# ChenFengYe/motion-latent-diffusion

Hardware: NVIDIA H100
Metric: motions/sec @ 50-step DDIM text-to-motion, batch 256 (higher is better)
Workload: dtype f16x2-split (fp32-equivalent, fp32 accumulate)

## Files before the change

mld_b200/csrc/gemm_tc.cu:

```cuda
#include "gemm_tc.h"

#include <algorithm>

#include "tc_common.cuh"

namespace {
using namespace tc;

constexpr int BM = 128, BK = 64;
constexpr int NUM_THREADS = 384;
constexpr int MMA_THREADS = 256;
constexpr int CONSUMER_WARPS = 8;
constexpr int MAX_N = 1024;
constexpr int MAX_N_WIDE = 4096;

struct TcParams {
  int M, N, kblocks, kb1;
  int m_tiles, n_tiles;
  float inv_scale;
  const float* bias;
  const float* addtab;
  int act;
  __half* out_hi; __half* out_lo; int ld_out, out_col0;
  float* out_f32; int ldc;
// ... 348 lines not shown
};

__global__ void __launch_bounds__(MMA_THREADS, 1)
k_ffn_tc(const __grid_constant__ CUtensorMap tmXh, const __grid_constant__ CUtensorMap tmXl,
         const __grid_constant__ CUtensorMap tmW1h, const __grid_constant__ CUtensorMap tmW1l,
         const __grid_constant__ CUtensorMap tmW2h, const __grid_constant__ CUtensorMap tmW2l,
         const __grid_constant__ CUtensorMap tmAh, const __grid_constant__ CUtensorMap tmAl,
         const __grid_constant__ CUtensorMap tmWoh, const __grid_constant__ CUtensorMap tmWol,
         const __grid_constant__ CUtensorMap tmYh, const __grid_constant__ CUtensorMap tmYl, const FfnParams p) {
  using Cfg = FfnCfg;
  constexpr int STAGES = Cfg::STAGES;
  extern __shared__ uint8_t smem_raw[];
  uint8_t* smem = smem_raw + smem_pad1024(smem_raw);
  uint8_t* ring = smem + Cfg::X_BYTES;
  uint64_t* bar_full = reinterpret_cast<uint64_t*>(ring + STAGES * Cfg::STAGE_BYTES);
  uint64_t* bar_empty = bar_full + STAGES;
  uint64_t* bar_xfull = bar_empty + STAGES;
  uint64_t* bar_xempty = bar_xfull + 4;

  const int warp = __shfl_sync(0xffffffffu, (int)(threadIdx.x >> 5), 0), lane = threadIdx.x & 31;
  int tl_n = 0;
  tl_event(p.tl, tl_n, 40);
  const int ncta = (int)gridDim.x, cid = (int)blockIdx.x;
  const int NC = p.n_chunks;
  struct Item { int mt, c0, c1, mode, piece0; };
  auto rev = [&](int t) { return p.reverse ? p.m_tiles - 1 - t : t; };
  const int nlocal = p.full + (cid < p.left * p.parts ? 1 : 0);
  auto item = [&](int j) -> Item {
    if (j < p.full) return Item{rev(cid + j * ncta), 0, NC, 0, 0};
    const int t = cid / p.parts, part = cid - t * p.parts;
    const int c0 = (part * NC + p.parts - 1) / p.parts, c1 = ((part + 1) * NC + p.parts - 1) / p.parts;
    const int slot0 = t * (p.parts - 1);
    return Item{rev(p.full * ncta + t), c0, c1, p.parts == 1 ? 0 : (part == p.parts - 1 ? 2 : 1),
                p.parts == 1 ? 0 : slot0 + (part == p.parts - 1 ? 0 : part)};
  };
  const int PRE = p.prefix ? 8 : 0;
  const int per_tile = PRE + 4 * NC;
  int total = p.full * per_tile;
  if (nlocal > p.full) {
    const Item it = item(p.full);
    total += PRE + 4 * (it.c1 - it.c0);
  }
  const int XG = p.prefix ? 2 : 1;
  const int xtotal = nlocal * 4 * XG;

  if (threadIdx.x == 0) {
    for (int s = 0; s < STAGES; ++s) {
      mbar_init(smem_u32(&bar_full[s]), 1);
      mbar_init(smem_u32(&bar_empty[s]), CONSUMER_WARPS);
    }
    for (int kb = 0; kb < 4; ++kb) {
      mbar_init(smem_u32(&bar_xfull[kb]), 1);
      mbar_init(smem_u32(&bar_xempty[kb]), CONSUMER_WARPS);
    }
    asm volatile("fence.mbarrier_init.release.cluster;" ::: "memory");
    tma_prefetch_desc(&tmXh); tma_prefetch_desc(&tmXl); tma_prefetch_desc(&tmW1h);
    tma_prefetch_desc(&tmW1l); tma_prefetch_desc(&tmW2h); tma_prefetch_desc(&tmW2l);
    tma_prefetch_desc(&tmYh); tma_prefetch_desc(&tmYl);
    if (p.prefix) { tma_prefetch_desc(&tmAh); tma_prefetch_desc(&tmAl); tma_prefetch_desc(&tmWoh); tma_prefetch_desc(&tmWol); }
  }
  pdl_trigger();
  __syncthreads();
  pdl_wait();
  tl_event(p.tl, tl_n, 41);

  int q_next = 0, x_next = 0;
  auto load_slot = [&](int q) {
    const int j = min(q / per_tile, p.full);
    const Item it = item(j);
    const int r = q - j * per_tile;
    if (elect_one()) {
      const uint32_t full = smem_u32(&bar_full[q % STAGES]);
      const uint32_t dst = smem_u32(ring + (q % STAGES) * Cfg::STAGE_BYTES);
      mbar_expect_tx(full, Cfg::STAGE_BYTES);
      if (r < PRE) {
        tma_load_2d(dst, (r & 1) ? &tmWol : &tmWoh, full, (r >> 1) * BK, 0);
      } else {
        const int c = it.c0 + ((r - PRE) >> 2), k = (r - PRE) & 3;
        if (k < 2) {
          for (int kk = 0; kk < 2; ++kk) {
            tma_load_2d(dst + kk * 8192, &tmW1h, full, (2 * k + kk) * BK, c * Cfg::CHUNK);
            tma_load_2d(dst + 16384 + kk * 8192, &tmW1l, full, (2 * k + kk) * BK, c * Cfg::CHUNK);
          }
        } else {
          tma_load_2d(dst, k == 3 ? &tmW2l : &tmW2h, full, c * Cfg::CHUNK, 0);
        }
      }
    }
    __syncwarp();
  };
  auto load_x = [&](int v) {
    if (elect_one()) {
      const int j = v / (4 * XG), kb = v & 3;
      const bool att = p.prefix && (v >> 2) == j * XG;
      const int m0 = item(j).mt * BM;
      const uint32_t full = smem_u32(&bar_xfull[kb]);
      mbar_expect_tx(full, 2 * BM * 128);
      tma_load_2d(smem_u32(smem + kb * 16384), att ? &tmAh : &tmXh, full, kb * BK, m0);
      tma_load_2d(smem_u32(smem + 65536 + kb * 16384), att ? &tmAl : &tmXl, full, kb * BK, m0);
      if (att && kb == 0)
        for (int k2 = 0; k2 < 4; ++k2) { tma_prefetch_2d(&tmXh, k2 * BK, m0); tma_prefetch_2d(&tmXl, k2 * BK, m0); }
      if (v % (4 * XG) == 0 && j + 1 < nlocal) {
        const int m1 = item(j + 1).mt * BM;
        for (int k2 = 0; k2 < 4; ++k2) {
          tma_prefetch_2d(&tmXh, k2 * BK, m1); tma_prefetch_2d(&tmXl, k2 * BK, m1);
          if (p.prefix) { tma_prefetch_2d(&tmAh, k2 * BK, m1); tma_prefetch_2d(&tmAl, k2 * BK, m1); }
        }
      }
    }
    __syncwarp();
  };
  auto produce = [&](int need, int need_x) {
    ring_produce(x_next, xtotal, need_x, bar_xempty, 4, load_x);
    ring_produce(q_next, total, need, bar_empty, STAGES, load_slot);
  };

  const int cw = warp >> 2;
  const int cp = 2 * (lane & 3);
  const int rl = cw * 64 + (warp & 3) * 16 + (lane >> 2);
  const uint32_t sX = smem_u32(smem) + cw * (64 * 128);
  float acc2[128];
  float acc1[32];
  uint32_t hh[4][4], hl[4][4];
  int rc = 0;
  auto slot_full = [&](int r) { mbar_wait(smem_u32(&bar_full[r % STAGES]), ((uint32_t)(r / STAGES)) & 1u); };
  auto slot_free = [&](int r) { if (lane == 0) mbar_arrive(smem_u32(&bar_empty[r % STAGES])); };
  auto x_full = [&](int kb, uint32_t par) { mbar_wait(smem_u32(&bar_xfull[kb]), par); };
  auto x_free = [&](int kb) { if (lane == 0) mbar_arrive(smem_u32(&bar_xempty[kb])); };
  for (int j = 0; j < nlocal; ++j) {
    const Item it = item(j);
    const int m0 = it.mt * BM;
    const uint32_t xpar = (uint32_t)(j * XG) & 1u;
    if (warp == 0) produce(-1, 4 * j * XG + 3);
    if (p.prefix) {
#pragma unroll
      for (int kb = 0; kb < 4; ++kb) {
        if (warp == 0) produce(rc + 1, -1);
        x_full(kb, xpar);
        slot_full(rc); slot_full(rc + 1);
        const uint32_t wh = smem_u32(ring + (rc % STAGES) * Cfg::STAGE_BYTES);
        const uint32_t wl = smem_u32(ring + ((rc + 1) % STAGES) * Cfg::STAGE_BYTES);
        wg_fence();
        kblock_ss<256>(acc2, sX + kb * 16384, sX + 65536 + kb * 16384, wh, wl, kb == 0);
        wg_commit();
        wg_wait<0>();
        slot_free(rc); slot_free(rc + 1); x_free(kb);
        rc += 2;
        if (warp == 0) produce(-1, -1);
        tl_event(p.tl, tl_n, 60, kb);
      }
      acc_fence(acc2);
      if (warp == 0) produce(-1, 4 * j * XG + 7);
#pragma unroll
      for (int kb = 0; kb < 4; ++kb) x_full(kb, xpar ^ 1u);
      ln_tile(acc2, p.inv_s0, p.b0, p.gamma1, p.beta1, smem, rl, lane, cp);
      fence_async_smem();
      named_bar_sync(2 + cw, 128);
      tl_event(p.tl, tl_n, 61, j);
    } else {
#pragma unroll
      for (int kb = 0; kb < 4; ++kb) x_full(kb, xpar);
    }
    tl_event(p.tl, tl_n, 2, j);
    int pend = -1;
    for (int c = it.c0; c < it.c1; ++c) {
#pragma unroll
      for (int half = 0; half < 2; ++half) {
        if (warp == 0) produce(rc + half, -1);
        slot_full(rc + half);
        tl_event(p.tl, tl_n, 10 + half, c);
        const uint32_t w = smem_u32(ring + ((rc + half) % STAGES) * Cfg::STAGE_BYTES);
        wg_fence();
#pragma unroll
        for (int k = 0; k < 2; ++k) {
          const uint32_t xh = sX + (2 * half + k) * 16384;
          kblock_ss<64>(acc1, xh, xh + 65536, w + k * 8192, w + 16384 + k * 8192, half == 0 && k == 0);
        }
        wg_commit();
      }
      wg_wait<0>();
      acc_fence(acc1);
      tl_event(p.tl, tl_n, 13, c);
      if (pend >= 0) slot_free(pend);
      slot_free(rc); slot_free(rc + 1);
      rc += 2;
      if (c == it.c1 - 1 && it.mode == 1)
        for (int kb = 0; kb < 4; ++kb) x_free(kb);
      if (warp == 0) produce(-1, -1);
#pragma unroll
      for (int ks = 0; ks < 4; ++ks) {
#pragma unroll
        for (int g = 0; g < 2; ++g) {
          const int jj = 2 * ks + g, n = c * Cfg::CHUNK + 8 * jj + cp;
          const float2 b = p.b1 ? __ldg(reinterpret_cast<const float2*>(p.b1 + n)) : make_float2(0.0f, 0.0f);
          split2(gelu_fast(fmaf(acc1[4 * jj], p.inv_s1, b.x)), gelu_fast(fmaf(acc1[4 * jj + 1], p.inv_s1, b.y)),
                 hh[ks][2 * g], hl[ks][2 * g]);
          split2(gelu_fast(fmaf(acc1[4 * jj + 2], p.inv_s1, b.x)), gelu_fast(fmaf(acc1[4 * jj + 3], p.inv_s1, b.y)),
                 hh[ks][2 * g + 1], hl[ks][2 * g + 1]);
        }
      }
      tl_event(p.tl, tl_n, 14, c);
      if (warp == 0) produce(rc, -1);
      slot_full(rc);
      tl_event(p.tl, tl_n, 12, c);
      wg_fence();
      {
        const uint64_t wd = make_desc(smem_u32(ring + (rc % STAGES) * Cfg::STAGE_BYTES));
#pragma unroll
        for (int ks = 0; ks < 4; ++ks) {
          wgmma_rs_n256(acc2, hl[ks], wd + 2 * ks, (c == it.c0 && ks == 0) ? 0u : 1u);
          wgmma_rs_n256(acc2, hh[ks], wd + 2 * ks, 1u);
        }
      }
      wg_commit();
      if (warp == 0) produce(rc + 1, -1);
      slot_full(rc + 1);
      {
        const uint64_t wd = make_desc(smem_u32(ring + ((rc + 1) % STAGES) * Cfg::STAGE_BYTES));
#pragma unroll
        for (int ks = 0; ks < 4; ++ks) wgmma_rs_n256(acc2, hh[ks], wd + 2 * ks, 1u);
      }
      wg_commit();
      wg_wait<1>();
      slot_free(rc);
      pend = rc + 1;
      rc += 2;
      if (warp == 0) produce(-1, -1);
    }
    wg_wait<0>();
    acc_fence(acc2);
    if (pend >= 0) slot_free(pend);
    if (warp == 0) produce(-1, -1);
    tl_event(p.tl, tl_n, 4, j);
    if (it.mode == 1) {
      float* const dst = p.scratch + (size_t)it.piece0 * (BM * 256);
#pragma unroll
      for (int jj = 0; jj < 32; ++jj) {
        *reinterpret_cast<float2*>(dst + rl * 256 + 8 * jj + cp) = make_float2(acc2[4 * jj], acc2[4 * jj + 1]);
        *reinterpret_cast<float2*>(dst + (rl + 8) * 256 + 8 * jj + cp) = make_float2(acc2[4 * jj + 2], acc2[4 * jj + 3]);
      }
      __threadfence();
      named_bar_sync(1, MMA_THREADS);
      if (threadIdx.x == 0) asm volatile("st.release.gpu.global.u32 [%0], %1;" ::"l"(p.flags + it.piece0), "r"(1) : "memory");
      continue;
    }
    const int nparts = it.mode == 2 ? p.parts - 1 : 0;
    if (nparts > 0) {
      if (lane == 0) {
        for (int pp = 0; pp < nparts; ++pp) {
          const int* f = p.flags + it.piece0 + pp;
          uint32_t v = 0;
          long long t_end = clock64() + 4000000000ll;
          do {
            asm volatile("ld.acquire.gpu.global.u32 %0, [%1];" : "=r"(v) : "l"(f) : "memory");
            if (v == 0 && clock64() > t_end) __trap();
          } while (v == 0);
        }
      }
      __syncwarp();
      for (int pp = 0; pp < nparts; ++pp) {
        const float* src = p.scratch + (size_t)(it.piece0 + pp) * (BM * 256);
#pragma unroll
        for (int jj = 0; jj < 32; ++jj) {
          const float2 a = __ldcg(reinterpret_cast<const float2*>(src + rl * 256 + 8 * jj + cp));
          const float2 b = __ldcg(reinterpret_cast<const float2*>(src + (rl + 8) * 256 + 8 * jj + cp));
          acc2[4 * jj] += a.x; acc2[4 * jj + 1] += a.y; acc2[4 * jj + 2] += b.x; acc2[4 * jj + 3] += b.y;
        }
      }
      named_bar_sync(1, MMA_THREADS);
      if (threadIdx.x == 0)
        for (int pp = 0; pp < nparts; ++pp) p.flags[it.piece0 + pp] = 0;
    }
    ln_tile(acc2, p.inv_s2, p.b2, p.gamma, p.beta, smem, rl, lane, cp);
    fence_async_smem();
    named_bar_sync(2 + cw, 128);
    tl_event(p.tl, tl_n, 62, j);
    if ((warp & 3) == 0) {
      if (elect_one()) {
        if (m0 + cw * 64 < p.M) {
#pragma unroll
          for (int kb = 0; kb < 4; ++kb) {
            const uint32_t src = smem_u32(smem + kb * 16384 + cw * 8192);
            tma_store_2d(&tmYh, src, kb * BK, m0 + cw * 64);
            tma_store_2d(&tmYl, src + 65536, kb * BK, m0 + cw * 64);
          }
          bulk_commit();
          bulk_wait_read<0>();
        }
#pragma unroll
        for (int kb = 0; kb < 4; ++kb) mbar_arrive_cnt(smem_u32(&bar_xempty[kb]), 4);
      }
      __syncwarp();
      tl_event(p.tl, tl_n, 63, j);
    }
  }
  tl_event(p.tl, tl_n, 42);
}

struct ProjParams {
  int M, n_chunks, items;
  float inv_scale;
  const float* bias;
  __half* out_hi; __half* out_lo; int ld_out, out_col0;
  long long* tl;
};
struct ProjCfg {
  static constexpr int CHUNK = 128;
  static constexpr int A_BYTES = 2 * 4 * BM * 128;
  static constexpr int STAGE_BYTES = 2 * CHUNK * 128, STAGES = 3;
  static constexpr int SMEM_BYTES = A_BYTES + STAGES * STAGE_BYTES + 256 + 1024;
  static_assert(SMEM_BYTES <= 232448, "shared memory budget");
};

template <int ACT>
__global__ void __launch_bounds__(MMA_THREADS, 1)
k_proj_tc(const __grid_constant__ CUtensorMap tmAh, const __grid_constant__ CUtensorMap tmAl,
          const __grid_constant__ CUtensorMap tmWh, const __grid_constant__ CUtensorMap tmWl, const ProjParams p) {
  using Cfg = ProjCfg;
  constexpr int STAGES = Cfg::STAGES;
  extern __shared__ uint8_t smem_raw[];
  uint8_t* smem = smem_raw + smem_pad1024(smem_raw);
  uint8_t* ring = smem + Cfg::A_BYTES;
  uint64_t* bar_full = reinterpret_cast<uint64_t*>(ring + STAGES * Cfg::STAGE_BYTES);
  uint64_t* bar_empty = bar_full + STAGES;
  uint64_t* bar_afull = bar_empty + STAGES;
  uint64_t* bar_aempty = bar_afull + 4;

  const int warp = __shfl_sync(0xffffffffu, (int)(threadIdx.x >> 5), 0), lane = threadIdx.x & 31;
  int tl_n = 0;
  tl_event(p.tl, tl_n, 40);
  const int NC = p.n_chunks;
  const int t0 = (int)((long long)blockIdx.x * p.items / gridDim.x);
  const int n = (int)((long long)(blockIdx.x + 1) * p.items / gridDim.x) - t0;
  const int mt0 = t0 / NC, ntiles = (t0 + n - 1) / NC - mt0 + 1;
  auto tile_of = [&](int i) { return (t0 + i) / NC - mt0; };
  auto first_of_tile = [&](int i) { return i == 0 || (t0 + i) % NC == 0; };
  auto last_of_tile = [&](int i) { return i == n - 1 || (t0 + i + 1) % NC == 0; };

  if (threadIdx.x == 0) {
    for (int s = 0; s < STAGES; ++s) {
      mbar_init(smem_u32(&bar_full[s]), 1);
      mbar_init(smem_u32(&bar_empty[s]), CONSUMER_WARPS);
    }
    for (int k = 0; k < 4; ++k) {
      mbar_init(smem_u32(&bar_afull[k]), 1);
      mbar_init(smem_u32(&bar_aempty[k]), CONSUMER_WARPS);
    }
    asm volatile("fence.mbarrier_init.release.cluster;" ::: "memory");
    tma_prefetch_desc(&tmAh); tma_prefetch_desc(&tmAl); tma_prefetch_desc(&tmWh); tma_prefetch_desc(&tmWl);
  }
  pdl_trigger();
  __syncthreads();
  pdl_wait();
  tl_event(p.tl, tl_n, 41);

  int q_next = 0, a_next = 0;
  auto load_w = [&](int q) {
    if (elect_one()) {
      const int c = (t0 + (q >> 2)) % NC, k = q & 3;
      const uint32_t full = smem_u32(&bar_full[q % STAGES]);
      const uint32_t dst = smem_u32(ring + (q % STAGES) * Cfg::STAGE_BYTES);
      mbar_expect_tx(full, Cfg::STAGE_BYTES);
      tma_load_2d(dst, &tmWh, full, k * BK, c * Cfg::CHUNK);
      tma_load_2d(dst + Cfg::STAGE_BYTES / 2, &tmWl, full, k * BK, c * Cfg::CHUNK);
    }
    __syncwarp();
  };
  auto load_a = [&](int a) {
    if (elect_one()) {
      const int j = a >> 2, k = a & 3, m0 = (mt0 + j) * BM;
      const uint32_t full = smem_u32(&bar_afull[k]);
      mbar_expect_tx(full, 2 * BM * 128);
      tma_load_2d(smem_u32(smem + k * 16384), &tmAh, full, k * BK, m0);
      tma_load_2d(smem_u32(smem + 65536 + k * 16384), &tmAl, full, k * BK, m0);
      if (k == 0 && j + 1 < ntiles)
        for (int k2 = 0; k2 < 4; ++k2) { tma_prefetch_2d(&tmAh, k2 * BK, m0 + BM); tma_prefetch_2d(&tmAl, k2 * BK, m0 + BM); }
    }
    __syncwarp();
  };
  auto produce = [&](int need_w, int need_a) {
    ring_produce(a_next, 4 * ntiles, need_a, bar_aempty, 4, load_a);
    ring_produce(q_next, 4 * n, need_w, bar_empty, STAGES, load_w);
  };

  const int cw = warp >> 2;
  const int cp = 2 * (lane & 3);
  const uint32_t sA = smem_u32(smem) + cw * (64 * 128);
  float acc0[64], acc1[64];
  auto retire = [&](int q) {
    if (lane == 0) {
      mbar_arrive(smem_u32(&bar_empty[q % STAGES]));
      if (last_of_tile(q >> 2)) mbar_arrive(smem_u32(&bar_aempty[q & 3]));
    }
  };
  auto epilogue = [&](const float (&d)[64], int i) {
    const int t = t0 + i, r_lo = (t / NC) * BM + cw * 64 + (warp & 3) * 16 + (lane >> 2), n0 = (t % NC) * Cfg::CHUNK;
    const int l = lane & 3;
    const bool ok0 = r_lo < p.M, ok1 = r_lo + 8 < p.M;
    const int64_t o0 = (int64_t)r_lo * p.ld_out + p.out_col0 + n0 + 8 * l, o1 = o0 + (int64_t)8 * p.ld_out;
    tl_event(p.tl, tl_n, 52, i);
#pragma unroll
    for (int jb = 0; jb < Cfg::CHUNK / 32; ++jb) {
      uint32_t h0[4], l0[4], h1[4], l1[4];
#pragma unroll
      for (int g = 0; g < 4; ++g) {
        const int j = 4 * jb + g;
        float x[4];
        fast_group<ACT>(d, j, p.inv_scale, __ldg(reinterpret_cast<const float2*>(p.bias + n0 + 8 * j + cp)), x);
        split2(x[0], x[1], h0[g], l0[g]);
        split2(x[2], x[3], h1[g], l1[g]);
      }
      quad_transpose(h0, l); quad_transpose(l0, l); quad_transpose(h1, l); quad_transpose(l1, l);
      if (ok0) {
        *reinterpret_cast<uint4*>(p.out_hi + o0 + 32 * jb) = make_uint4(h0[0], h0[1], h0[2], h0[3]);
        *reinterpret_cast<uint4*>(p.out_lo + o0 + 32 * jb) = make_uint4(l0[0], l0[1], l0[2], l0[3]);
      }
      if (ok1) {
        *reinterpret_cast<uint4*>(p.out_hi + o1 + 32 * jb) = make_uint4(h1[0], h1[1], h1[2], h1[3]);
        *reinterpret_cast<uint4*>(p.out_lo + o1 + 32 * jb) = make_uint4(l1[0], l1[1], l1[2], l1[3]);
      }
    }
    tl_event(p.tl, tl_n, 53, i);
  };
  auto step = [&](int i, float (&cur)[64], float (&prev)[64]) {
    const bool fresh = first_of_tile(i);
    const int j = tile_of(i);
    tl_event(p.tl, tl_n, 50, i);
#pragma unroll
    for (int k = 0; k < 4; ++k) {
      const int q = 4 * i + k;
      if (warp == 0) produce(q, fresh ? 4 * j + k : -1);
      if (fresh) {
        mbar_wait(smem_u32(&bar_afull[k]), (uint32_t)j & 1u);
        if (k == 0) tl_event(p.tl, tl_n, 51, j);
      }
      mbar_wait(smem_u32(&bar_full[q % STAGES]), ((uint32_t)(q / STAGES)) & 1u);
      const uint32_t w = smem_u32(ring + (q % STAGES) * Cfg::STAGE_BYTES), a = sA + k * 16384;
      wg_fence();
      kblock_ss<128>(cur, a, a + 65536, w, w + Cfg::STAGE_BYTES / 2, k == 0);
      wg_commit();
      if (k == 2) {
        if (warp == 0) produce(q + 1, -1);
        if (i > 0) epilogue(prev, i - 1);
      }
      if (q > 0) {
        wg_wait<1>();
        retire(q - 1);
      }
      if (k == 0 && i > 0) acc_fence(prev);
    }
  };
  for (int i = 0; i < n; i += 2) {
    step(i, acc0, acc1);
    if (i + 1 < n) step(i + 1, acc1, acc0);
  }
  wg_wait<0>();
  retire(4 * n - 1);
  if ((n - 1) & 1) {
    acc_fence(acc1);
    epilogue(acc1, n - 1);
  } else {
    acc_fence(acc0);
    epilogue(acc0, n - 1);
  }
  tl_event(p.tl, tl_n, 42);
}

}

struct TcCtx {
  int device = 0;
  int sm_count = 132;
  int ffn_fused = 1;
  int ffn_split = 1;
};

TcCtx* tc_create(int device) {
  if (!tc::tmap_encoder()) return nullptr;
  TcCtx* c = new TcCtx();
  c->device = device;
  cudaDeviceGetAttribute(&c->sm_count, cudaDevAttrMultiProcessorCount, device);
  bool ok = true;
  auto opt_in = [&](auto kernel, int bytes) { ok = ok && smem_opt_in(kernel, bytes, "k_gemm_tc"); };
  opt_in(k_gemm_tc<256, EPI_FAST>, TileCfg<256>::SMEM_BYTES); opt_in(k_gemm_tc<128, EPI_FAST>, TileCfg<128>::SMEM_BYTES);
  opt_in(k_gemm_tc<256, EPI_FAST, ACT_GELU>, TileCfg<256>::SMEM_BYTES); opt_in(k_gemm_tc<128, EPI_FAST, ACT_GELU>, TileCfg<128>::SMEM_BYTES);
  opt_in(k_gemm_tc<256, EPI_GENERIC>, TileCfg<256>::SMEM_BYTES); opt_in(k_gemm_tc<128, EPI_GENERIC>, TileCfg<128>::SMEM_BYTES);
  opt_in(k_gemm_tc<256, EPI_FAST, ACT_QUICKGELU>, TileCfg<256>::SMEM_BYTES);
  opt_in(k_gemm_tc<128, EPI_FAST, ACT_QUICKGELU>, TileCfg<128>::SMEM_BYTES);
  opt_in(k_gemm_tc<256, EPI_RES>, TileCfg<256>::SMEM_BYTES); opt_in(k_gemm_tc<128, EPI_RES>, TileCfg<128>::SMEM_BYTES);
  opt_in(k_gemm_tc<256, EPI_LN>, TileCfg<256>::SMEM_BYTES);
  opt_in(k_gemm_tc<256, EPI_FAST, ACT_LEAKY>, TileCfg<256>::SMEM_BYTES); opt_in(k_gemm_tc<128, EPI_FAST, ACT_LEAKY>, TileCfg<128>::SMEM_BYTES);
  opt_in(k_gemm_tc<256, EPI_F32>, TileCfg<256>::SMEM_BYTES); opt_in(k_gemm_tc<128, EPI_F32>, TileCfg<128>::SMEM_BYTES);
  opt_in(k_gemm_tc<256, EPI_F32, ACT_LEAKY>, TileCfg<256>::SMEM_BYTES); opt_in(k_gemm_tc<128, EPI_F32, ACT_LEAKY>, TileCfg<128>::SMEM_BYTES);
  opt_in(k_ffn_tc, FfnCfg::SMEM_BYTES);
  opt_in(k_proj_tc<ACT_NONE>, ProjCfg::SMEM_BYTES); opt_in(k_proj_tc<ACT_GELU>, ProjCfg::SMEM_BYTES);
  opt_in(k_proj_tc<ACT_QUICKGELU>, ProjCfg::SMEM_BYTES); opt_in(k_proj_tc<ACT_LEAKY>, ProjCfg::SMEM_BYTES);
  if (!ok) {
    delete c;
    return nullptr;
  }
  return c;
}
void tc_destroy(TcCtx* c) { delete c; }

static int pick_bn(const GemmArgs& g) { return (g.w.N % 256 == 0) ? 256 : 128; }

bool tc_gemm_supported(const TcCtx* c, const GemmArgs& g) {
  if (!c) return false;
  if (g.a_kind != A_SPLIT || g.M < 1 || g.w.N > (g.wide_n ? MAX_N_WIDE : MAX_N)) return false;
  if (g.K1 <= 0 || g.K1 % BK || g.K2 % BK || g.a1.cols != g.K1) return false;
  if (g.K2 > 0 && g.a2.cols != g.K2) return false;
  if (g.w.K != g.K1 + g.K2) return false;
  if (((uintptr_t)g.a1.hi & 15) || ((uintptr_t)g.w.w & 15)) return false;
  if (g.out.hi && ((g.out.cols % 8) || (g.out_col0 % 8))) return false;
  if (g.res_f32 && (!g.out_f32 || g.out.hi || g.act != ACT_NONE || g.addtab || g.zero_lengths || g.in_group < g.M ||
                    g.out_group != 0 || g.out_off != 0 || (g.w.N % 2) || (g.ldc % 2) || ((uintptr_t)g.out_f32 & 7) ||
                    ((uintptr_t)g.res_f32 & 7)))
    return false;
  return true;
}

bool tc_gemm_ln_supported(const TcCtx* c, const GemmArgs& g, const LnArgs& l) {
  if (!tc_gemm_supported(c, g)) return false;
  if (g.w.N != 256 || l.d != 256 || g.act != ACT_NONE) return false;
  if (l.in_group != 0 || l.c != nullptr || l.out_f32 != nullptr || !l.out.hi) return false;
  if (l.out.cols != 256 || (l.res.hi && l.res.cols != 256)) return false;
  if (l.gamma2 || l.rowvec) return false;
  if (g.addtab || g.zero_lengths || g.in_group < g.M || g.out_group != 0 || g.out_off != 0) return false;
  return true;
}

static void fill_params(const GemmArgs& g, const LnArgs* ln, int bn, TcParams* out) {
  TcParams p{};
  p.M = g.M; p.N = g.w.N; p.kblocks = g.w.K / BK; p.kb1 = g.K1 / BK;
  p.inv_scale = g.w.inv_scale; p.bias = g.w.bias; p.addtab = g.addtab; p.act = g.act;
  p.in_group = g.in_group; p.out_group = g.out_group; p.out_off = g.out_off; p.zero_lengths = g.zero_lengths;
  if (ln) {
    p.out_hi = ln->out.hi; p.out_lo = ln->out.lo(); p.ld_out = ln->out.cols; p.out_col0 = 0;
    p.res_hi = ln->res.hi; p.res_lo = ln->res.hi ? ln->res.lo() : nullptr; p.ld_res = ln->res.cols;
    p.gamma = ln->gamma; p.beta = ln->beta;
  } else {
    p.out_hi = g.out.hi; p.out_lo = g.out.hi ? g.out.lo() : nullptr; p.ld_out = g.out.cols; p.out_col0 = g.out_col0;
    p.out_f32 = g.out_f32; p.ldc = g.ldc; p.res_f32 = g.res_f32;
  }
  p.m_tiles = (g.M + BM - 1) / BM;
  p.n_tiles = (g.w.N + bn - 1) / bn;
  p.tl = tc::mldb_timeline_buffer();
  *out = p;
}

static bool tc_proj(TcCtx* c, const GemmArgs& g, cudaStream_t st) {
  CUtensorMap mAh, mAl, mWh, mWl;
  const bool ok = make_map(&mAh, g.a1.hi, g.M, g.K1, BM) && make_map(&mAl, g.a1.lo(), g.M, g.K1, BM) &&
                  make_map(&mWh, g.w.w, g.w.N, g.w.K, ProjCfg::CHUNK) &&
                  make_map(&mWl, g.w.w + g.w.plane_stride, g.w.N, g.w.K, ProjCfg::CHUNK);
  if (!ok) return false;
  ProjParams p{};
  p.M = g.M; p.n_chunks = g.w.N / ProjCfg::CHUNK; p.items = (g.M + BM - 1) / BM * p.n_chunks;
  p.inv_scale = g.w.inv_scale; p.bias = g.w.bias;
  p.out_hi = g.out.hi; p.out_lo = g.out.lo(); p.ld_out = g.out.cols; p.out_col0 = g.out_col0;
  p.tl = tc::mldb_timeline_buffer();
  const dim3 grid(p.items < c->sm_count ? p.items : c->sm_count);
  switch (g.act) {
    case ACT_GELU: launch_pdl(k_proj_tc<ACT_GELU>, grid, dim3(MMA_THREADS), ProjCfg::SMEM_BYTES, st, mAh, mAl, mWh, mWl, p); break;
    case ACT_QUICKGELU: launch_pdl(k_proj_tc<ACT_QUICKGELU>, grid, dim3(MMA_THREADS), ProjCfg::SMEM_BYTES, st, mAh, mAl, mWh, mWl, p); break;
    case ACT_LEAKY: launch_pdl(k_proj_tc<ACT_LEAKY>, grid, dim3(MMA_THREADS), ProjCfg::SMEM_BYTES, st, mAh, mAl, mWh, mWl, p); break;
    default: launch_pdl(k_proj_tc<ACT_NONE>, grid, dim3(MMA_THREADS), ProjCfg::SMEM_BYTES, st, mAh, mAl, mWh, mWl, p); break;
  }
  return true;
}

bool tc_gemm(TcCtx* c, const GemmArgs& g, const LnArgs* ln, cudaStream_t st) {
  const int bn = ln ? 256 : pick_bn(g);
  const bool fast = !ln && g.out.hi && !g.out_f32 && !g.addtab && !g.zero_lengths && g.in_group >= g.M &&
                    g.out_group == 0 && g.out_off == 0 && g.w.N % bn == 0 && g.w.bias != nullptr &&
                    (g.act == ACT_NONE || g.act == ACT_GELU || g.act == ACT_QUICKGELU || g.act == ACT_LEAKY);
  if (fast && g.K1 == 256 && g.K2 == 0 && ((uintptr_t)g.out.hi & 15) == 0 && ((uintptr_t)g.out.lo() & 15) == 0)
    return tc_proj(c, g, st);
  CUtensorMap mA1h, mA1l, mA2h, mA2l, mWh, mWl;
  bool ok = make_map(&mA1h, g.a1.hi, g.M, g.K1, BM) && make_map(&mA1l, g.a1.lo(), g.M, g.K1, BM);
  if (g.K2 > 0) ok = ok && make_map(&mA2h, g.a2.hi, g.M, g.K2, BM) && make_map(&mA2l, g.a2.lo(), g.M, g.K2, BM);
  else { mA2h = mA1h; mA2l = mA1l; }
  ok = ok && make_map(&mWh, g.w.w, g.w.N, g.w.K, bn) && make_map(&mWl, g.w.w + g.w.plane_stride, g.w.N, g.w.K, bn);
  if (!ok) return false;
  TcParams p;
  fill_params(g, ln, bn, &p);
  const bool f32 = !ln && g.vec_f32 && !g.out.hi && g.out_f32 && !g.res_f32 && !g.addtab && !g.zero_lengths &&
                   g.in_group >= g.M && g.out_group == 0 && g.out_off == 0 && g.w.N % 2 == 0 && g.ldc % 2 == 0 &&
                   ((uintptr_t)g.out_f32 & 7) == 0 && (g.act == ACT_NONE || g.act == ACT_LEAKY);
  const int ntiles = p.m_tiles * p.n_tiles;
  dim3 grid(ntiles < c->sm_count ? ntiles : c->sm_count);
#define MLDB_LAUNCH(BN_, ...)                                                                                      \
  launch_pdl(k_gemm_tc<BN_, __VA_ARGS__>, grid, dim3(NUM_THREADS), TileCfg<BN_>::SMEM_BYTES, st, mA1h, mA1l, mA2h, \
             mA2l, mWh, mWl, p)
#define MLDB_LAUNCH_SHAPE(...)                                                       \
  do {                                                                               \
    if (bn == 256) MLDB_LAUNCH(256, __VA_ARGS__); else MLDB_LAUNCH(128, __VA_ARGS__); \
  } while (0)
  if (ln)                             MLDB_LAUNCH(256, EPI_LN);
  else if (g.res_f32)                 MLDB_LAUNCH_SHAPE(EPI_RES);
  else if (fast && g.act == ACT_GELU) MLDB_LAUNCH_SHAPE(EPI_FAST, ACT_GELU);
  else if (fast && g.act == ACT_QUICKGELU) MLDB_LAUNCH_SHAPE(EPI_FAST, ACT_QUICKGELU);
  else if (fast && g.act == ACT_LEAKY) MLDB_LAUNCH_SHAPE(EPI_FAST, ACT_LEAKY);
  else if (f32 && g.act == ACT_LEAKY) MLDB_LAUNCH_SHAPE(EPI_F32, ACT_LEAKY);
  else if (f32)                       MLDB_LAUNCH_SHAPE(EPI_F32);
  else if (fast)                      MLDB_LAUNCH_SHAPE(EPI_FAST);
  else                                MLDB_LAUNCH_SHAPE(EPI_GENERIC);
#undef MLDB_LAUNCH_SHAPE
#undef MLDB_LAUNCH
  return true;
}

int tc_set_ffn_split(TcCtx* c, int on) {
  if (!c) return 0;
  const int old = c->ffn_split;
  c->ffn_split = on;
  return old;
}
int tc_set_ffn_fused(TcCtx* c, int on) {
  if (!c) return 0;
  const int old = c->ffn_fused;
  c->ffn_fused = on;
  return old;
}
static bool planes_aligned16(const ActBuf& b) { return ((uintptr_t)b.hi & 15) == 0 && ((uintptr_t)b.lo() & 15) == 0; }

bool tc_ffn_supported(const TcCtx* c, const GemmArgs& g1, const GemmArgs& g2, const LnArgs& l2) {
  if (!c || !c->ffn_fused) return false;
  if (!tc_gemm_supported(c, g1) || !tc_gemm_ln_supported(c, g2, l2)) return false;
  if (g1.K1 != 256 || g1.K2 > 0 || g2.K2 > 0 || g1.M != g2.M) return false;
  if (g1.w.N % FfnCfg::CHUNK || g1.w.N > MAX_N || g1.w.N != g2.K1) return false;
  if (g1.act != ACT_GELU || g1.out_f32 || g1.addtab || g1.zero_lengths) return false;
  if (g1.in_group < g1.M || g1.out_group != 0 || g1.out_off != 0) return false;
  if (l2.res.hi != g1.a1.hi || l2.res.plane_stride != g1.a1.plane_stride) return false;
  if (!planes_aligned16(g1.a1) || !planes_aligned16(l2.out)) return false;
  return true;
}
bool tc_tail_supported(const TcCtx* c, const GemmArgs& go, const LnArgs& l1, const GemmArgs& g1, const GemmArgs& g2,
                       const LnArgs& l2) {
  if (!tc_gemm_ln_supported(c, go, l1) || !tc_ffn_supported(c, g1, g2, l2)) return false;
  if (go.K1 != 256 || go.K2 > 0 || go.M != g1.M || !l1.res.hi) return false;
  if (g1.a1.hi != l1.out.hi || g1.a1.plane_stride != l1.out.plane_stride) return false;
  return planes_aligned16(go.a1) && planes_aligned16(l1.res);
}

static bool launch_ffn(TcCtx* c, const GemmArgs* go, const LnArgs* l1, const GemmArgs& g1, const GemmArgs& g2,
                       const LnArgs& l2, float* scratch, int* flags, cudaStream_t st) {
  CUtensorMap mXh, mXl, mW1h, mW1l, mW2h, mW2l, mAh, mAl, mWoh, mWol, mYh, mYl;
  const int M = g1.M, m_tiles = (M + BM - 1) / BM;
  const ActBuf x = go ? l1->res : g1.a1;
  bool ok = make_map(&mXh, x.hi, M, 256, BM) && make_map(&mXl, x.lo(), M, 256, BM) &&
            make_map(&mW1h, g1.w.w, g1.w.N, g1.w.K, FfnCfg::CHUNK) &&
            make_map(&mW1l, g1.w.w + g1.w.plane_stride, g1.w.N, g1.w.K, FfnCfg::CHUNK) &&
            make_map(&mW2h, g2.w.w, g2.w.N, g2.w.K, 256) &&
            make_map(&mW2l, g2.w.w + g2.w.plane_stride, g2.w.N, g2.w.K, 256) &&
            make_map(&mYh, l2.out.hi, M, 256, 64) && make_map(&mYl, l2.out.lo(), M, 256, 64);
  if (go) {
    ok = ok && make_map(&mAh, go->a1.hi, M, 256, BM) && make_map(&mAl, go->a1.lo(), M, 256, BM) &&
         make_map(&mWoh, go->w.w, go->w.N, go->w.K, 256) && make_map(&mWol, go->w.w + go->w.plane_stride, go->w.N, go->w.K, 256);
  } else {
    mAh = mXh; mAl = mXl; mWoh = mW2h; mWol = mW2l;
  }
  if (!ok) return false;
  FfnParams p{};
  p.M = M; p.m_tiles = m_tiles; p.n_chunks = g1.w.N / FfnCfg::CHUNK;
  p.tl = tc::mldb_timeline_buffer();
  p.prefix = go ? 1 : 0;
  if (go) { p.inv_s0 = go->w.inv_scale; p.b0 = go->w.bias; p.gamma1 = l1->gamma; p.beta1 = l1->beta; }
  p.inv_s1 = g1.w.inv_scale; p.inv_s2 = g2.w.inv_scale;
  p.b1 = g1.w.bias; p.b2 = g2.w.bias; p.gamma = l2.gamma; p.beta = l2.beta;
  const int ncta_max = c->sm_count;
  p.full = m_tiles / ncta_max; p.left = m_tiles % ncta_max; p.parts = 1;
  p.scratch = scratch; p.flags = flags;
  if (p.left > 0 && scratch && flags && c->ffn_split) {
    const int parts = std::min(p.n_chunks, ncta_max / p.left);
    if (parts >= 2 && (size_t)p.left * (parts - 1) * (BM * 256 * 4) <= TC_FFN_SCRATCH_BYTES) p.parts = parts;
  }
  const int ncta = p.full > 0 ? ncta_max : p.left * p.parts;
  p.reverse = tc::snake_order();
  launch_pdl(k_ffn_tc, dim3(ncta), dim3(MMA_THREADS), FfnCfg::SMEM_BYTES, st, mXh, mXl, mW1h, mW1l, mW2h, mW2l, mAh,
             mAl, mWoh, mWol, mYh, mYl, p);
  return true;
}
bool tc_ffn(TcCtx* c, const GemmArgs& g1, const GemmArgs& g2, const LnArgs& l2, float* scratch, int* flags, cudaStream_t st) {
  return launch_ffn(c, nullptr, nullptr, g1, g2, l2, scratch, flags, st);
}
bool tc_tail(TcCtx* c, const GemmArgs& go, const LnArgs& l1, const GemmArgs& g1, const GemmArgs& g2, const LnArgs& l2,
             float* scratch, int* flags, cudaStream_t st) {
  return launch_ffn(c, &go, &l1, g1, g2, l2, scratch, flags, st);
}
```

Before: 860.9.

## Route N=256 GEMM+LayerNorm through projection kernel with fused residual LN epilogue

Adds an LN mode to the projection kernel. Each CTA computes a full 128x256 row tile as two 128-column chunks into a 128-float accumulator. The epilogue adds bias and the split-half residual, then applies LayerNorm and writes the split outputs, with L2 prefetch of the next tile's residual rows. GEMM+LN calls with K=256 and N=256 now take this lighter 256-thread path instead of the generic 384-thread k_gemm_tc EPI_LN kernel. The cost is higher register pressure from the 128-register accumulator and less tile parallelism, since each CTA owns whole rows.

```diff
diff --git a/mld_b200/csrc/gemm_tc.cu b/mld_b200/csrc/gemm_tc.cu
--- a/mld_b200/csrc/gemm_tc.cu
+++ b/mld_b200/csrc/gemm_tc.cu
@@ -674,6 +674,8 @@
   float inv_scale;
   const float* bias;
   __half* out_hi; __half* out_lo; int ld_out, out_col0;
+  const __half* res_hi; const __half* res_lo; int ld_res;
+  const float* gamma; const float* beta;
   long long* tl;
 };
 struct ProjCfg {
@@ -684,10 +686,10 @@
   static_assert(SMEM_BYTES <= 232448, "shared memory budget");
 };
 
-template <int ACT>
-__global__ void __launch_bounds__(MMA_THREADS, 1)
-k_proj_tc(const __grid_constant__ CUtensorMap tmAh, const __grid_constant__ CUtensorMap tmAl,
-          const __grid_constant__ CUtensorMap tmWh, const __grid_constant__ CUtensorMap tmWl, const ProjParams p) {
+template <int ACT, bool LN>
+__device__ __forceinline__ void proj_tc(const CUtensorMap& tmAh, const CUtensorMap& tmAl, const CUtensorMap& tmWh,
+                                        const CUtensorMap& tmWl, const ProjParams& p) {
+  static_assert(!LN || ACT == ACT_NONE, "the LayerNorm mode has no activation");
   using Cfg = ProjCfg;
   constexpr int STAGES = Cfg::STAGES;
   extern __shared__ uint8_t smem_raw[];
@@ -702,12 +704,14 @@
   int tl_n = 0;
   tl_event(p.tl, tl_n, 40);
   const int NC = p.n_chunks;
+  const int IPT = LN ? 1 : NC;
+  constexpr int PER = LN ? 8 : 4;
   const int t0 = (int)((long long)blockIdx.x * p.items / gridDim.x);
   const int n = (int)((long long)(blockIdx.x + 1) * p.items / gridDim.x) - t0;
-  const int mt0 = t0 / NC, ntiles = (t0 + n - 1) / NC - mt0 + 1;
-  auto tile_of = [&](int i) { return (t0 + i) / NC - mt0; };
-  auto first_of_tile = [&](int i) { return i == 0 || (t0 + i) % NC == 0; };
-  auto last_of_tile = [&](int i) { return i == n - 1 || (t0 + i + 1) % NC == 0; };
+  const int mt0 = t0 / IPT, ntiles = (t0 + n - 1) / IPT - mt0 + 1;
+  auto tile_of = [&](int i) { return (t0 + i) / IPT - mt0; };
+  auto first_of_tile = [&](int i) { return i == 0 || (t0 + i) % IPT == 0; };
+  auto last_of_tile = [&](int i) { return i == n - 1 || (t0 + i + 1) % IPT == 0; };
 
   if (threadIdx.x == 0) {
     for (int s = 0; s < STAGES; ++s) {
@@ -729,7 +733,7 @@
   int q_next = 0, a_next = 0;
   auto load_w = [&](int q) {
     if (elect_one()) {
-      const int c = (t0 + (q >> 2)) % NC, k = q & 3;
+      const int c = LN ? (q >> 2) & 1 : (t0 + (q >> 2)) % NC, k = q & 3;
       const uint32_t full = smem_u32(&bar_full[q % STAGES]);
       const uint32_t dst = smem_u32(ring + (q % STAGES) * Cfg::STAGE_BYTES);
       mbar_expect_tx(full, Cfg::STAGE_BYTES);
@@ -752,19 +756,110 @@
   };
   auto produce = [&](int need_w, int need_a) {
     ring_produce(a_next, 4 * ntiles, need_a, bar_aempty, 4, load_a);
-    ring_produce(q_next, 4 * n, need_w, bar_empty, STAGES, load_w);
+    ring_produce(q_next, PER * n, need_w, bar_empty, STAGES, load_w);
   };
 
   const int cw = warp >> 2;
   const int cp = 2 * (lane & 3);
   const uint32_t sA = smem_u32(smem) + cw * (64 * 128);
-  float acc0[64], acc1[64];
+  float acc[128];
+  float (&acc0)[64] = *reinterpret_cast<float (*)[64]>(acc);
+  float (&acc1)[64] = *reinterpret_cast<float (*)[64]>(acc + 64);
   auto retire = [&](int q) {
     if (lane == 0) {
       mbar_arrive(smem_u32(&bar_empty[q % STAGES]));
-      if (last_of_tile(q >> 2)) mbar_arrive(smem_u32(&bar_aempty[q & 3]));
+      if (LN ? ((q >> 2) & 1) != 0 : last_of_tile(q >> 2)) mbar_arrive(smem_u32(&bar_aempty[q & 3]));
     }
   };
+  if constexpr (LN) {
+    auto chunk = [&](int i, int c, float (&cur)[64]) {
+#pragma unroll
+      for (int k = 0; k < 4; ++k) {
+        const int q = 8 * i + 4 * c + k;
+        if (warp == 0) produce(q, c == 0 ? 4 * i + k : -1);
+        if (c == 0) {
+          mbar_wait(smem_u32(&bar_afull[k]), (uint32_t)i & 1u);
+          if (k == 0) tl_event(p.tl, tl_n, 51, i);
+        }
+        mbar_wait(smem_u32(&bar_full[q % STAGES]), ((uint32_t)(q / STAGES)) & 1u);
+        const uint32_t w = smem_u32(ring + (q % STAGES) * Cfg::STAGE_BYTES), a = sA + k * 16384;
+        wg_fence();
+        kblock_ss<128>(cur, a, a + 65536, w, w + Cfg::STAGE_BYTES / 2, k == 0);
+        wg_commit();
+        if (c > 0 || k > 0) {
+          wg_wait<1>();
+          retire(q - 1);
+        }
+      }
+    };
+    const int l = lane & 3;
+    auto prefetch_res = [&](int i) {
+      const int r = (t0 + i) * BM + cw * 64 + (warp & 3) * 16 + (lane >> 2);
+#pragma unroll
+      for (int h = 0; h < 2; ++h)
+        if (r + 8 * h < p.M) {
+          const int64_t o = (int64_t)(r + 8 * h) * p.ld_res + 64 * l;
+          asm volatile("prefetch.global.L2 [%0];" ::"l"(p.res_hi + o));
+          asm volatile("prefetch.global.L2 [%0];" ::"l"(p.res_lo + o));
+        }
+    };
+    prefetch_res(0);
+    for (int i = 0; i < n; ++i) {
+      tl_event(p.tl, tl_n, 50, i);
+      chunk(i, 0, acc0);
+      chunk(i, 1, acc1);
+      wg_wait<0>();
+      acc_fence(acc);
+      retire(8 * i + 7);
+      tl_event(p.tl, tl_n, 4, i);
+      if (warp == 0) produce(8 * (i + 1) + 2, 4 * (i + 1) + 3);
+      if (i + 1 < n) prefetch_res(i + 1);
+      tl_event(p.tl, tl_n, 54, i);
+      const int r_lo = (t0 + i) * BM + cw * 64 + (warp & 3) * 16 + (lane >> 2);
+      const bool ok0 = r_lo < p.M, ok1 = r_lo + 8 < p.M;
+      const int64_t ro0 = (int64_t)r_lo * p.ld_res + 8 * l, ro1 = ro0 + (int64_t)8 * p.ld_res;
+      const int64_t o0 = (int64_t)r_lo * p.ld_out + 8 * l, o1 = o0 + (int64_t)8 * p.ld_out;
+      uint32_t h0[4], l0[4], h1[4], l1[4];
+      auto load16 = [](const __half* src, bool ok, uint32_t (&v)[4]) {
+        const uint4 u = ok ? *reinterpret_cast<const uint4*>(src) : make_uint4(0u, 0u, 0u, 0u);
+        v[0] = u.x; v[1] = u.y; v[2] = u.z; v[3] = u.w;
+      };
+      ln_rows(acc, p.inv_scale, p.bias, p.gamma, p.beta, cp,
+              [&](int j, float (&x)[4]) {
+                const int g = j & 3, jb = j >> 2;
+                if (g == 0) {
+                  load16(p.res_hi + ro0 + 32 * jb, ok0, h0); load16(p.res_lo + ro0 + 32 * jb, ok0, l0);
+                  load16(p.res_hi + ro1 + 32 * jb, ok1, h1); load16(p.res_lo + ro1 + 32 * jb, ok1, l1);
+                  quad_transpose(h0, l); quad_transpose(l0, l); quad_transpose(h1, l); quad_transpose(l1, l);
+                }
+                const float2 a0 = __half22float2(*reinterpret_cast<const __half2*>(&h0[g]));
+                const float2 b0 = __half22float2(*reinterpret_cast<const __half2*>(&l0[g]));
+                const float2 a1 = __half22float2(*reinterpret_cast<const __half2*>(&h1[g]));
+                const float2 b1 = __half22float2(*reinterpret_cast<const __half2*>(&l1[g]));
+                if (ok0) { x[0] = (x[0] + a0.x) + b0.x; x[1] = (x[1] + a0.y) + b0.y; }
+                if (ok1) { x[2] = (x[2] + a1.x) + b1.x; x[3] = (x[3] + a1.y) + b1.y; }
+              },
+              [&](int j, const float (&y)[4]) {
+                const int g = j & 3, jb = j >> 2;
+                split2(y[0], y[1], h0[g], l0[g]);
+                split2(y[2], y[3], h1[g], l1[g]);
+                if (g == 3) {
+                  quad_transpose(h0, l); quad_transpose(l0, l); quad_transpose(h1, l); quad_transpose(l1, l);
+                  if (ok0) {
+                    *reinterpret_cast<uint4*>(p.out_hi + o0 + 32 * jb) = make_uint4(h0[0], h0[1], h0[2], h0[3]);
+                    *reinterpret_cast<uint4*>(p.out_lo + o0 + 32 * jb) = make_uint4(l0[0], l0[1], l0[2], l0[3]);
+                  }
+                  if (ok1) {
+                    *reinterpret_cast<uint4*>(p.out_hi + o1 + 32 * jb) = make_uint4(h1[0], h1[1], h1[2], h1[3]);
+                    *reinterpret_cast<uint4*>(p.out_lo + o1 + 32 * jb) = make_uint4(l1[0], l1[1], l1[2], l1[3]);
+                  }
+                }
+              });
+      tl_event(p.tl, tl_n, 55, i);
+    }
+    tl_event(p.tl, tl_n, 42);
+    return;
+  }
   auto epilogue = [&](const float (&d)[64], int i) {
     const int t = t0 + i, r_lo = (t / NC) * BM + cw * 64 + (warp & 3) * 16 + (lane >> 2), n0 = (t % NC) * Cfg::CHUNK;
     const int l = lane & 3;
@@ -836,6 +931,18 @@
     epilogue(acc0, n - 1);
   }
   tl_event(p.tl, tl_n, 42);
+}
+
+template <int ACT>
+__global__ void __launch_bounds__(MMA_THREADS, 1)
+k_proj_tc(const __grid_constant__ CUtensorMap tmAh, const __grid_constant__ CUtensorMap tmAl,
+          const __grid_constant__ CUtensorMap tmWh, const __grid_constant__ CUtensorMap tmWl, const ProjParams p) {
+  proj_tc<ACT, false>(tmAh, tmAl, tmWh, tmWl, p);
+}
+__global__ void __launch_bounds__(MMA_THREADS, 1)
+k_proj_ln_tc(const __grid_constant__ CUtensorMap tmAh, const __grid_constant__ CUtensorMap tmAl,
+             const __grid_constant__ CUtensorMap tmWh, const __grid_constant__ CUtensorMap tmWl, const ProjParams p) {
+  proj_tc<ACT_NONE, true>(tmAh, tmAl, tmWh, tmWl, p);
 }
 
 }
@@ -867,6 +974,7 @@
   opt_in(k_ffn_tc, FfnCfg::SMEM_BYTES);
   opt_in(k_proj_tc<ACT_NONE>, ProjCfg::SMEM_BYTES); opt_in(k_proj_tc<ACT_GELU>, ProjCfg::SMEM_BYTES);
   opt_in(k_proj_tc<ACT_QUICKGELU>, ProjCfg::SMEM_BYTES); opt_in(k_proj_tc<ACT_LEAKY>, ProjCfg::SMEM_BYTES);
+  opt_in(k_proj_ln_tc, ProjCfg::SMEM_BYTES);
   if (!ok) {
     delete c;
     return nullptr;
@@ -921,18 +1029,28 @@
   *out = p;
 }
 
-static bool tc_proj(TcCtx* c, const GemmArgs& g, cudaStream_t st) {
+static bool planes_aligned16(const ActBuf& b) { return ((uintptr_t)b.hi & 15) == 0 && ((uintptr_t)b.lo() & 15) == 0; }
+
+static bool tc_proj(TcCtx* c, const GemmArgs& g, const LnArgs* ln, cudaStream_t st) {
   CUtensorMap mAh, mAl, mWh, mWl;
   const bool ok = make_map(&mAh, g.a1.hi, g.M, g.K1, BM) && make_map(&mAl, g.a1.lo(), g.M, g.K1, BM) &&
-                  make_map(&mWh, g.w.w, g.w.N, g.w.K, ProjCfg::CHUNK) &&
-                  make_map(&mWl, g.w.w + g.w.plane_stride, g.w.N, g.w.K, ProjCfg::CHUNK);
+            make_map(&mWh, g.w.w, g.w.N, g.w.K, ProjCfg::CHUNK) &&
+            make_map(&mWl, g.w.w + g.w.plane_stride, g.w.N, g.w.K, ProjCfg::CHUNK);
   if (!ok) return false;
   ProjParams p{};
-  p.M = g.M; p.n_chunks = g.w.N / ProjCfg::CHUNK; p.items = (g.M + BM - 1) / BM * p.n_chunks;
+  p.M = g.M; p.n_chunks = g.w.N / ProjCfg::CHUNK;
+  p.items = (g.M + BM - 1) / BM * (ln ? 1 : p.n_chunks);
   p.inv_scale = g.w.inv_scale; p.bias = g.w.bias;
-  p.out_hi = g.out.hi; p.out_lo = g.out.lo(); p.ld_out = g.out.cols; p.out_col0 = g.out_col0;
   p.tl = tc::mldb_timeline_buffer();
   const dim3 grid(p.items < c->sm_count ? p.items : c->sm_count);
+  if (ln) {
+    p.out_hi = ln->out.hi; p.out_lo = ln->out.lo(); p.ld_out = ln->out.cols;
+    p.res_hi = ln->res.hi; p.res_lo = ln->res.lo(); p.ld_res = ln->res.cols;
+    p.gamma = ln->gamma; p.beta = ln->beta;
+    launch_pdl(k_proj_ln_tc, grid, dim3(MMA_THREADS), ProjCfg::SMEM_BYTES, st, mAh, mAl, mWh, mWl, p);
+    return true;
+  }
+  p.out_hi = g.out.hi; p.out_lo = g.out.lo(); p.ld_out = g.out.cols; p.out_col0 = g.out_col0;
   switch (g.act) {
     case ACT_GELU: launch_pdl(k_proj_tc<ACT_GELU>, grid, dim3(MMA_THREADS), ProjCfg::SMEM_BYTES, st, mAh, mAl, mWh, mWl, p); break;
     case ACT_QUICKGELU: launch_pdl(k_proj_tc<ACT_QUICKGELU>, grid, dim3(MMA_THREADS), ProjCfg::SMEM_BYTES, st, mAh, mAl, mWh, mWl, p); break;
@@ -948,7 +1066,10 @@
                     g.out_group == 0 && g.out_off == 0 && g.w.N % bn == 0 && g.w.bias != nullptr &&
                     (g.act == ACT_NONE || g.act == ACT_GELU || g.act == ACT_QUICKGELU || g.act == ACT_LEAKY);
   if (fast && g.K1 == 256 && g.K2 == 0 && ((uintptr_t)g.out.hi & 15) == 0 && ((uintptr_t)g.out.lo() & 15) == 0)
-    return tc_proj(c, g, st);
+    return tc_proj(c, g, nullptr, st);
+  if (ln && g.K1 == 256 && g.K2 == 0 && g.w.N == 256 && ln->res.hi && planes_aligned16(ln->res) &&
+      planes_aligned16(ln->out))
+    return tc_proj(c, g, ln, st);
   CUtensorMap mA1h, mA1l, mA2h, mA2l, mWh, mWl;
   bool ok = make_map(&mA1h, g.a1.hi, g.M, g.K1, BM) && make_map(&mA1l, g.a1.lo(), g.M, g.K1, BM);
   if (g.K2 > 0) ok = ok && make_map(&mA2h, g.a2.hi, g.M, g.K2, BM) && make_map(&mA2l, g.a2.lo(), g.M, g.K2, BM);
@@ -995,8 +1116,6 @@
   c->ffn_fused = on;
   return old;
 }
-static bool planes_aligned16(const ActBuf& b) { return ((uintptr_t)b.hi & 15) == 0 && ((uintptr_t)b.lo() & 15) == 0; }
-
 bool tc_ffn_supported(const TcCtx* c, const GemmArgs& g1, const GemmArgs& g2, const LnArgs& l2) {
   if (!c || !c->ffn_fused) return false;
   if (!tc_gemm_supported(c, g1) || !tc_gemm_ln_supported(c, g2, l2)) return false;
```

Result: faster. 870.7 (median of 6 runs) (+1.1%).
